# IRFM/librir

Hardware: AMD Instinct MI355X
Metric: IR frames/sec encode+decode, 640x512 uint16 (higher is better)
Workload: dtype u16; 1 GPU; configs[1]: 1000-frame 640x512 uint16 stream (S1 noisy background, seed 1234+rank), lossless RIRB1 encode+decode, device-resident, GOP 50, per GPU; two launches per step: the encoder leaves the PACKED form (headers + position and length per segment + the payload without holes: encoded_footprint_bytes, in a buffer of half the raw size), the decoder reads it as it is; the compressed payload (17 % of; frames_per_gpu=1000, width=640, height=512, gop=50

## Files before the change

### librir_amd/csrc/codec_kernels.hip

```cpp
#include <hip/hip_runtime.h>
#include <algorithm>
#include <stdint.h>

#include "codec_format.h"
#include "filter_kernels.h"
#include "runtime.h"

namespace rir
{

	constexpr int FRAME_LOAD_AUX = 2;
	constexpr int FRAME_STORE_AUX = 2;
	constexpr int SPARSE_STORE_AUX = 0;
	constexpr int STREAM_LOAD_AUX = 0;

	typedef short short2v __attribute__((ext_vector_type(2)));
	typedef unsigned short ushort2v __attribute__((ext_vector_type(2)));

	__device__ __forceinline__ uint32_t pk_sub16(uint32_t a, uint32_t b)
	{
		return __builtin_bit_cast(uint32_t, __builtin_bit_cast(ushort2v, a) - __builtin_bit_cast(ushort2v, b));
	}
	__device__ __forceinline__ uint32_t pk_add16(uint32_t a, uint32_t b)
	{
// ... 306 lines not shown
		v = max(v, (uint32_t)__builtin_amdgcn_mov_dpp((int)v, 0x121, 0xf, 0xf, false));
		v = max(v, (uint32_t)__builtin_amdgcn_mov_dpp((int)v, 0x122, 0xf, 0xf, false));
		v = max(v, (uint32_t)__builtin_amdgcn_mov_dpp((int)v, 0x124, 0xf, 0xf, false));
		v = max(v, (uint32_t)__builtin_amdgcn_mov_dpp((int)v, 0x128, 0xf, 0xf, false));
		return v;
	}
	__device__ __forceinline__ uint32_t rows_inclusive_sum(uint32_t w)
	{
		const uint32_t s = w + (uint32_t)__builtin_amdgcn_update_dpp(0, (int)w, 0x142, 0xa, 0xf, false);
		return s + (uint32_t)__builtin_amdgcn_update_dpp(0, (int)s, 0x143, 0xc, 0xf, false);
	}

	__device__ __forceinline__ uint32_t half_inclusive_sum(uint32_t v)
	{
		v += (uint32_t)__builtin_amdgcn_update_dpp(0, (int)v, 0x111, 0xf, 0xf, true);
		v += (uint32_t)__builtin_amdgcn_update_dpp(0, (int)v, 0x112, 0xf, 0xf, true);
		v += (uint32_t)__builtin_amdgcn_update_dpp(0, (int)v, 0x114, 0xf, 0xf, true);
		v += (uint32_t)__builtin_amdgcn_update_dpp(0, (int)v, 0x118, 0xf, 0xf, true);
		v += (uint32_t)__builtin_amdgcn_update_dpp(0, (int)v, 0x142, 0xa, 0xf, false);
		return v;
	}
	__device__ __forceinline__ uint32_t bitlen_nz(uint32_t f) { return 31u - (uint32_t)__builtin_clz((f << 1) | 1u); }

	struct RecordWords
	{
		v2u32 va, vb;
		uint32_t pa, pb;
	};

	template <uint32_t SCALE, uint32_t NONE>
	__device__ __forceinline__ uint64_t emit_words_narrow(const Px8 &r, uint32_t mode, uint32_t base, RecordWords &rw, uint32_t pos,
														  const LaneConsts &lc, const TransposeConsts &tc, uint32_t *words)
	{
		uint32_t x = (r.d[0] | (r.d[1] << 8)) | ((r.d[2] | (r.d[3] << 8)) << 4);
		x = transpose32(x, tc);
		const uint64_t nz64 = __ballot(x != 0);
		const uint32_t nz = (uint32_t)nz64 | (uint32_t)(nz64 >> 32);
		uint32_t M = nz | ((nz >> 1) & 0x77777777u);
		M |= (M >> 2) & 0x33333333u;
		uint32_t W = M - ((M >> 1) & 0x55555555u);
		W = (W & 0x33333333u) + ((W >> 2) & 0x33333333u);
		*words = (uint32_t)__builtin_popcount(M);
		auto sw = __builtin_amdgcn_permlane32_swap(x, x, false, false);
		rw.va.x = x, rw.va.y = sw[1];
		const uint32_t at = (pos + (uint32_t)__builtin_popcount(M & lc.p_before)) * SCALE;
		rw.pa = __builtin_amdgcn_inverse_ballot_w64((uint64_t)M) ? at : NONE;
		rw.vb = rw.va, rw.pb = NONE;
		const uint32_t B = base | (mode << 16);
		const uint64_t hw = __ballot((int32_t)(W << lc.p_hshw) < 0) & 0x00E700E700E700E7ull;
		const uint64_t hb = __ballot((int32_t)(B << lc.p_hshb) < 0) & 0x3C003C003C00FC00ull;
		return hw | hb;
	}

	template <uint32_t SCALE, uint32_t NONE>
	__device__ __forceinline__ uint64_t emit_words_wide(const Px8 &r, uint32_t mode, uint32_t base, RecordWords &rw, uint32_t pos,
														const LaneConsts &lc, const TransposeConsts &tc, uint32_t *words)
	{
		uint32_t alo = r.d[0], ahi = r.d[1], blo = r.d[2], bhi = r.d[3];
		transpose64x2(alo, ahi, blo, bhi, tc);
		const uint32_t wa = row_allmax((alo | ahi) != 0 ? lc.bitp1 : 0u);
		const uint32_t wb = row_allmax((blo | bhi) != 0 ? lc.bitp1 : 0u);
		const uint32_t ia = rows_inclusive_sum(wa), ib = rows_inclusive_sum(wb);
		const uint32_t tot_a = (uint32_t)__builtin_amdgcn_readlane((int)ia, 63);
		const uint32_t tot_b = (uint32_t)__builtin_amdgcn_readlane((int)ib, 63);
		rw.va.x = alo, rw.va.y = ahi, rw.vb.x = blo, rw.vb.y = bhi;
		rw.pa = lc.bit < wa ? (pos + ia - wa + lc.bit) * SCALE : NONE;
		rw.pb = lc.bit < wb ? (pos + tot_a + ib - wb + lc.bit) * SCALE : NONE;
		*words = tot_a + tot_b;
		const uint32_t nib = (base >> lc.sh4) & 15u;
		const uint32_t field = ((nib << 10) | (lc.row0 ? mode << 14 : 0u)) | ((wb << 5) | wa);
		return __ballot((field & lc.onehot) != 0);
	}

	template <uint32_t SCALE, uint32_t NONE>
	__device__ __forceinline__ uint64_t emit_words(const Px8 &r, uint32_t mode, uint32_t base, RecordWords &rw, uint32_t pos, const LaneConsts &lc,
												   const TransposeConsts &tc, uint32_t *words)
	{
		const uint32_t any = (r.d[0] | r.d[1]) | (r.d[2] | r.d[3]);
		if (__ballot((any & 0xfff0fff0u) != 0) == 0)
			return emit_words_narrow<SCALE, NONE>(r, mode, base, rw, pos, lc, tc, words);
		return emit_words_wide<SCALE, NONE>(r, mode, base, rw, pos, lc, tc, words);
	}

	struct DirectSink
	{
		__amdgpu_buffer_rsrc_t out;
		template <int DIR>
		__device__ __forceinline__ uint64_t emit(const Px8 &r, uint32_t mode, uint32_t base, uint32_t pos, const LaneConsts &lc,
												 const TransposeConsts &tc, uint32_t *words)
		{
			static_assert(DIR > 0, "a slot is filled in frame order from word 0: the direct sink only walks forwards");
			RecordWords rw;
			const uint64_t h = emit_words<8u, RIR_OOB>(r, mode, base, rw, pos, lc, tc, words);
			__builtin_amdgcn_raw_buffer_store_b64(rw.va, out, rw.pa, 0, SPARSE_STORE_AUX);
			__builtin_amdgcn_raw_buffer_store_b64(rw.vb, out, rw.pb, 0, SPARSE_STORE_AUX);
			return h;
		}
	};

	__device__ __noinline__ uint64_t staging_take_extent(unsigned long long *cursor, uint32_t need, uint64_t arena_words, uint32_t *error_word)
	{
		unsigned long long off = 0;
		if ((threadIdx.x & 63u) == 0)
			off = __hip_atomic_fetch_add(cursor, (unsigned long long)need, __ATOMIC_RELAXED, __HIP_MEMORY_SCOPE_AGENT);
		const uint32_t lo = (uint32_t)__builtin_amdgcn_readfirstlane((int)(uint32_t)off);
		const uint32_t hi = (uint32_t)__builtin_amdgcn_readfirstlane((int)(uint32_t)(off >> 32));
		off = ((unsigned long long)hi << 32) | lo;
		if (off + need > arena_words)
		{
			if ((threadIdx.x & 63u) == 0)
				__hip_atomic_fetch_or(error_word, 2u, __ATOMIC_RELAXED, __HIP_MEMORY_SCOPE_AGENT);
			return ~0ull;
		}
		return off;
	}

	struct Staging
	{
		uint64_t *lds;
		uint32_t cap;
		uint32_t lds_used;
		bool spilling;
		__amdgpu_buffer_rsrc_t spill;
		uint32_t need;
		uint64_t *arena;
		unsigned long long *cursor;
		uint64_t arena_words;
		uint64_t extent;
		uint32_t *error_word;

		__device__ __forceinline__ Staging(uint64_t *lds_all, int w, int cap_, int nrec)
			: lds(lds_all + (size_t)w * cap_), cap((uint32_t)cap_), lds_used(0), spilling(false), need((uint32_t)(nrec > 0 ? nrec : 0) * RIRB1_REC_MAX_WORDS),
			  arena(nullptr), cursor(nullptr), arena_words(0), extent(~0ull), error_word(nullptr)
		{
		}

		template <int DIR>
		__device__ __forceinline__ uint64_t emit(const Px8 &r, uint32_t mode, uint32_t base, uint32_t pos, const LaneConsts &lc, const TransposeConsts &tc,
												 uint32_t *words)
		{
			RecordWords rw;
			const uint64_t h = emit_words<1u, RIR_NONE>(r, mode, base, rw, DIR > 0 ? pos : 0u, lc, tc, words);
			if (!spilling && pos + *words > cap)
			{
				spilling = true, lds_used = pos;
				if (arena)
				{
					const uint64_t ext = staging_take_extent(cursor, need, arena_words, error_word);
					extent = ((uint64_t)(uint32_t)__builtin_amdgcn_readfirstlane((int)(uint32_t)(ext >> 32)) << 32) |
							 (uint32_t)__builtin_amdgcn_readfirstlane((int)(uint32_t)ext);
					if (extent != ~0ull)
						spill = make_rsrc(arena + extent, need * 8u);
				}
			}
			if (!spilling)
			{
				uint64_t *rec = DIR > 0 ? lds : lds + (cap - pos - *words);
				if (rw.pa != RIR_NONE)
					rec[rw.pa] = ((uint64_t)rw.va.y << 32) | rw.va.x;
				if (rw.pb != RIR_NONE)
					rec[rw.pb] = ((uint64_t)rw.vb.y << 32) | rw.vb.x;
			}
			const uint32_t add = !spilling ? RIR_OOB : DIR > 0 ? 0u - lds_used * 8u : (need - (pos - lds_used) - *words) * 8u;
			const uint32_t oa = rw.pa != RIR_NONE ? rw.pa * 8u + add : RIR_OOB;
			const uint32_t ob = rw.pb != RIR_NONE ? rw.pb * 8u + add : RIR_OOB;
			__builtin_amdgcn_raw_buffer_store_b64(rw.va, spill, oa, 0, SPARSE_STORE_AUX);
			__builtin_amdgcn_raw_buffer_store_b64(rw.vb, spill, ob, 0, SPARSE_STORE_AUX);
			return h;
		}
	};

	template <bool FAST, int DIR, class Sink>
	__device__ __forceinline__ uint32_t encode_run(const uint16_t *__restrict__ frames, int64_t npx, int nload, int64_t frame_first, bool has_key,
												   int tile, int lane, uint64_t *__restrict__ hdr_first, Sink &sink)
	{
		constexpr bool BACK = DIR < 0;
		const int64_t p0 = (int64_t)tile * RIRB1_TILE_PX + lane * 8;
		const TransposeConsts tc = make_transpose_consts(lane);
		const LaneConsts lc = make_lane_consts(lane);
		const uint32_t lane_off = (uint32_t)lane * 16u;
		const uint16_t *next_ptr = frames + (frame_first + (BACK ? nload - 1 : 0)) * npx + (int64_t)tile * RIRB1_TILE_PX;
		auto load = [&](int k, v4u32 &dst) {
			if (FAST)
			{
				const Px8 p = buf_load8(next_ptr, k < nload ? lane_off : RIR_OOB);
				dst.x = p.d[0], dst.y = p.d[1], dst.z = p.d[2], dst.w = p.d[3];
				next_ptr = BACK ? next_ptr - npx : next_ptr + npx;
			}
			else
			{
				const int i = min(k, nload - 1);
				const Px8 p = load8(frames, frame_first + (BACK ? nload - 1 - i : i), npx, p0, false);
				dst.x = p.d[0], dst.y = p.d[1], dst.z = p.d[2], dst.w = p.d[3];
			}
		};
		auto as_px8 = [](const v4u32 &v) {
			Px8 p;
			p.d[0] = v.x, p.d[1] = v.y, p.d[2] = v.z, p.d[3] = v.w;
			return p;
		};
		uint32_t pos = 0;
		uint64_t hdr_reg = 0;
		auto key_record = [&](const Px8 &cur) {
			const uint32_t base_raw = tile_base(cur, false);
			const uint32_t b2 = base_raw | (base_raw << 16);
			Px8 r_raw;
#pragma unroll
			for (int k = 0; k < 4; ++k)
				r_raw.d[k] = pk_sub16(cur.d[k], b2);
			const Px8 dl = left_delta(cur, lane);
			const uint32_t base_left = tile_base(dl, true);
			const uint32_t bl2 = base_left | (base_left << 16);
			Px8 r_left;
#pragma unroll
			for (int k = 0; k < 4; ++k)
				r_left.d[k] = pk_sub16(dl.d[k], bl2);
			const bool use_left = payload_words(r_left) < payload_words(r_raw);
			Px8 r_sel;
#pragma unroll
			for (int k = 0; k < 4; ++k)
				r_sel.d[k] = use_left ? r_left.d[k] : r_raw.d[k];
			uint32_t words;
			const uint32_t key_mode = use_left ? RIRB1_MODE_LEFT : RIRB1_MODE_RAW;
			const uint64_t h = sink.template emit<DIR>(r_sel, key_mode, use_left ? base_left : base_raw, pos, lc, tc, &words);
			if (lane == 0)
				hdr_first[0] = h;
			pos += words;
		};
		v4u32 s0, s1, s2, s3;
		load(0, s0);
		load(1, s1);
		load(2, s2);
		load(3, s3);
		if (!BACK && has_key)
			key_record(as_px8(s0));
#define RIR_ENC_STEP(K, NEW, OLD)                                                             \
	{                                                                                          \
		const int k_ = (K);                                                                    \
		Px8 d;                                                                                 \
		{                                                                                      \
			const Px8 c_ = as_px8(BACK ? OLD : NEW), p_ = as_px8(BACK ? NEW : OLD);            \
			_Pragma("unroll") for (int k = 0; k < 4; ++k) d.d[k] = pk_sub16(c_.d[k], p_.d[k]); \
		}                                                                                      \
		load(k_ + 3, OLD);                                                                     \
		const uint32_t base = tile_base(d, true);                                              \
		const uint32_t b2 = base | (base << 16);                                               \
		_Pragma("unroll") for (int k = 0; k < 4; ++k) d.d[k] = pk_sub16(d.d[k], b2);          \
		uint32_t words;                                                                        \
		const uint64_t h = sink.template emit<DIR>(d, RIRB1_MODE_TEMPORAL, base, pos, lc, tc, &words); \
		if (lane == ((k_ - 1) & 63))                                                           \
			hdr_reg = h;                                                                       \
		pos += words;                                                                          \
	}
		int fb = 1;
		while (fb < nload)
		{
			const int g0 = fb, gend = min(fb + 64, nload);
			for (; fb + 3 < gend; fb += 4)
			{
				RIR_ENC_STEP(fb, s1, s0)
				RIR_ENC_STEP(fb + 1, s2, s1)
				RIR_ENC_STEP(fb + 2, s3, s2)
				RIR_ENC_STEP(fb + 3, s0, s3)
			}
			if (fb < gend)
			{
				RIR_ENC_STEP(fb, s1, s0)
				if (fb + 1 < gend)
				{
					RIR_ENC_STEP(fb + 1, s2, s1)
					if (fb + 2 < gend)
						RIR_ENC_STEP(fb + 2, s3, s2)
				}
				fb = gend;
			}
			if (g0 + lane < gend)
				hdr_first[BACK ? nload - (g0 + lane) : g0 + lane] = hdr_reg;
			hdr_reg = 0;
		}
#undef RIR_ENC_STEP
		if (BACK && has_key)
		{
			const int ks = (nload - 1) & 3;
			const v4u32 kv = ks == 0 ? s0 : ks == 1 ? s1 : ks == 2 ? s2 : s3;
			key_record(as_px8(kv));
		}
		return pos;
	}

	template <bool FAST>
	__attribute__((amdgpu_waves_per_eu(8, 8))) __global__ __launch_bounds__(256) void rirb1_encode_tiles(const uint16_t *__restrict__ frames, int64_t npx, int ntiles,
																 int tile_first, int tile_count, int nframes, int gop,
																 uint64_t *__restrict__ hdr_table, uint32_t *__restrict__ seg_words,
																 uint64_t *__restrict__ sparse)
	{
		const int lane = threadIdx.x & 63;
		const int ti = blockIdx.x * 4 + __builtin_amdgcn_readfirstlane((int)(threadIdx.x >> 6));
		if (ti >= tile_count)
			return;
		const int tile = tile_first + ti;
		const int chunk = blockIdx.y;
		const int f_begin = chunk * gop;
		const int nf = min(gop, nframes - f_begin);
		const int64_t slot = (int64_t)chunk * ntiles + tile;
		uint64_t *my_hdr = hdr_table + slot * gop;
		DirectSink sink{make_rsrc(sparse + slot * RIRB1_SLOT_WORDS(gop), (uint32_t)gop * RIRB1_REC_MAX_WORDS * 8u)};
		const uint32_t words = encode_run<FAST, 1>(frames, npx, nf, f_begin, true, tile, lane, my_hdr, sink);
		for (int f = nf + lane; f < gop; f += 64)
			my_hdr[f] = 0;
		if (lane == 0)
			seg_words[slot] = words;
	}

	__global__ __launch_bounds__(256) void rirb1_scan_tiles(const uint32_t *__restrict__ seg_words, int ntiles,
														   uint32_t *__restrict__ tile_off, uint64_t *__restrict__ chunk_words)
	{
		__shared__ uint32_t wave_tot[4];
		__shared__ uint32_t carry_s;
		const int c = blockIdx.x, tid = threadIdx.x, lane = tid & 63, wv = tid >> 6;
		const uint32_t *in = seg_words + (int64_t)c * ntiles;
		uint32_t *off = tile_off + (int64_t)c * (ntiles + 1);
		if (tid == 0)
			carry_s = 0;
		__syncthreads();
		for (int base = 0; base < ntiles; base += 256)
		{
			const int i = base + tid;
			const uint32_t v = i < ntiles ? in[i] : 0u;
			const uint32_t inc = wave_scan_add(v, lane);
			if (lane == 63)
				wave_tot[wv] = inc;
			__syncthreads();
			uint32_t pre = carry_s;
			for (int k = 0; k < wv; ++k)
				pre += wave_tot[k];
			if (i < ntiles)
				off[i] = pre + inc - v;
			__syncthreads();
			if (tid == 255)
				carry_s = pre + inc;
			__syncthreads();
		}
		if (tid == 0)
		{
			off[ntiles] = carry_s;
			chunk_words[c] = carry_s;
		}
	}

	__global__ __launch_bounds__(256) void rirb1_compact(const uint64_t *__restrict__ sparse, const uint32_t *__restrict__ tile_off,
														const uint64_t *__restrict__ chunk_words, int ntiles, int nchunks, int gop,
														uint64_t *__restrict__ chunk_off, uint64_t *__restrict__ stream)
	{
		const int t = blockIdx.x, c = blockIdx.y, tid = threadIdx.x;
		const uint32_t *off = tile_off + (int64_t)c * (ntiles + 1);
		const uint32_t o0 = off[t], o1 = off[t + 1];
		uint64_t s = 0;
		for (int i = tid & 63; i < c; i += 64)
			s += chunk_words[i];
#pragma unroll
		for (int d = 32; d >= 1; d >>= 1)
			s += (uint64_t)__shfl_xor((long long)s, d, 64);
// ... 311 lines not shown
		const int f_begin = chunk * gop;
		const int nf = min(gop, nframes - f_begin);
		uint64_t *my_hdr = hdr_table + seg * gop;

		const WaveShare sh = wave_share<enc_split_mirrored>(w, WAVES, nf);
		Staging sg(enc_lds, w, cap, sh.nrec);
		sg.spill = make_rsrc(arena, 0);
		sg.arena = arena, sg.cursor = spill_cursor, sg.arena_words = arena_words, sg.error_word = error_word;
		uint32_t pos = 0;
		if (sh.nrec > 0)
		{
			if (enc_walks_back(w))
				pos = encode_run<FAST, -1>(frames, npx, sh.nload, (int64_t)f_begin + sh.first_load, sh.has_key, tile, lane, my_hdr + sh.first_load, sg);
			else
				pos = encode_run<FAST, 1>(frames, npx, sh.nload, (int64_t)f_begin + sh.first_load, sh.has_key, tile, lane, my_hdr + sh.first_load, sg);
		}
		if (lane == 0)
			sh_u64[1 + w] = sg.extent;
		staged_publish<WAVES>(my_hdr, nf, gop, sg, pos, w, lane, sh_u32, sh_u32 + WAVES);
		__syncthreads();
		if (w != 0)
			return;
		uint32_t total = 0;
		bool lost = false;
#pragma unroll
		for (int i = 0; i < WAVES; ++i)
		{
			const uint32_t n = sh_u32[i];
			total += n;
			lost |= n > sh_u32[WAVES + i] && sh_u64[1 + i] == ~0ull;
		}
		unsigned long long at = 0;
		if (lane == 0)
			at = __hip_atomic_fetch_add(cursor, (unsigned long long)total | (1ull << RIR_PACKED_COUNT_SHIFT), __ATOMIC_RELAXED, __HIP_MEMORY_SCOPE_AGENT);
		const uint32_t lo = (uint32_t)__builtin_amdgcn_readfirstlane((int)(uint32_t)at);
		const uint32_t hi = (uint32_t)__builtin_amdgcn_readfirstlane((int)(uint32_t)(at >> 32));
		const uint32_t arrived = hi >> (RIR_PACKED_COUNT_SHIFT - 32);
		const uint64_t nseg = (uint64_t)gridDim.y * (uint32_t)ntiles;
		const uint64_t on_side = downwards ? nseg / 2 : (nseg + 1) / 2;
		if ((uint64_t)arrived + 1 == on_side)
			packed_finish(ctrl, capacity_words, nseg < 2 ? 1u : 2u);
		at = ((unsigned long long)hi << 32 | lo) & RIR_PACKED_WORDS_MASK;
		const bool fits = at + total <= capacity_words;
		if (downwards)
			at = capacity_words - at - total;
		if (lane == 0)
		{
			seg_pos[seg] = at;
			seg_words[seg] = total;
			sh_u64[0] = (fits && !lost) ? at : ~0ull;
		}
		if (!fits || lost)
			return;
		uint64_t *dst = stream + at;
		for (int i = 0; i < WAVES; ++i)
		{
			const uint32_t n_all = sh_u32[i];
			copy_wave_words(dst, enc_lds + (size_t)i * cap, (uint32_t)cap, n_all, sh_u32[WAVES + i], enc_walks_back(i), lane, [&](uint32_t &need) {
				need = (uint32_t)wave_share<enc_split_mirrored>(i, WAVES, nf).nrec * RIRB1_REC_MAX_WORDS;
				return make_rsrc(arena + sh_u64[1 + i], need * 8u);
			});
			dst += n_all;
		}
	}

	struct Fetched
	{
		uint64_t hdr;
		v2u32 a, b;
		uint32_t words;
		bool bad;
		bool narrow;
	};

	__device__ __forceinline__ bool header_is_narrow(uint64_t hdr)
	{
		const uint64_t m0 = 0x0021002100210021ull;
		const uint64_t hi = hdr & (m0 * 0x18u);
		const uint64_t b2 = (hdr >> 2) & m0;
		const uint64_t lo = (hdr | (hdr >> 1)) & m0;
		return (hi | (b2 & lo)) == 0;
	}

	__device__ __forceinline__ Fetched fetch_record(uint64_t hdr, __amdgpu_buffer_rsrc_t in, uint32_t pos, uint32_t seg_len, const LaneConsts &lc)
	{
		Fetched r;
		r.hdr = hdr;
		r.narrow = header_is_narrow(hdr);
		const bool hdr_bad = ((hdr & 0xC000C000C0000000ull) != 0) || (((hdr >> 14) & 3u) == 3u);
		uint32_t oa, ob;
		if (r.narrow)
		{
			const uint32_t w = ((lc.n_hhi ? (uint32_t)(hdr >> 32) : (uint32_t)hdr) >> lc.n_hsh) & 31u;
			const uint32_t incl = half_inclusive_sum(lc.n_first ? w : 0u);
			r.words = (uint32_t)__builtin_amdgcn_readlane((int)incl, 31);
			r.bad = hdr_bad || (pos + r.words > seg_len);
			oa = (!r.bad && lc.n_half == 0 && lc.n_bit < w) ? (pos + incl - w + lc.n_bit) * 8u : RIR_OOB;
			ob = RIR_OOB;
		}
		else
		{
			const uint32_t field = ((lc.row_hi ? (uint32_t)(hdr >> 32) : (uint32_t)hdr) >> lc.sh16) & 0xffffu;
			const uint32_t wa = field & 31u, wb = (field >> 5) & 31u;
			const uint32_t ia = rows_inclusive_sum(wa), ib = rows_inclusive_sum(wb);
			const uint32_t tot_a = (uint32_t)__builtin_amdgcn_readlane((int)ia, 63);
			const uint32_t tot_b = (uint32_t)__builtin_amdgcn_readlane((int)ib, 63);
			r.words = tot_a + tot_b;
			const bool too_wide = __ballot(wa > 16u || wb > 16u) != 0;
			r.bad = hdr_bad || too_wide || (pos + r.words > seg_len);
			oa = (!r.bad && lc.bit < wa) ? (pos + ia - wa + lc.bit) * 8u : RIR_OOB;
			ob = (!r.bad && lc.bit < wb) ? (pos + tot_a + ib - wb + lc.bit) * 8u : RIR_OOB;
		}
		r.a = __builtin_amdgcn_raw_buffer_load_b64(in, oa, 0, STREAM_LOAD_AUX);
		r.b = __builtin_amdgcn_raw_buffer_load_b64(in, ob, 0, STREAM_LOAD_AUX);
		return r;
	}

	__device__ __forceinline__ Px8 planes_to_residuals(v2u32 a, v2u32 b, bool narrow, const TransposeConsts &tc)
	{
		Px8 r;
		if (narrow)
		{
			auto sw = __builtin_amdgcn_permlane32_swap(a.x, a.y, false, false);
			const uint32_t x = transpose32(sw[0], tc);
			const uint32_t lo = x & 0x0f0f0f0fu, hi = (x >> 4) & 0x0f0f0f0fu;
			r.d[0] = __builtin_amdgcn_perm(hi, lo, 0x0c040c00u);
			r.d[1] = __builtin_amdgcn_perm(hi, lo, 0x0c050c01u);
			r.d[2] = __builtin_amdgcn_perm(hi, lo, 0x0c060c02u);
			r.d[3] = __builtin_amdgcn_perm(hi, lo, 0x0c070c03u);
		}
		else
		{
			uint32_t alo = a.x, ahi = a.y, blo = b.x, bhi = b.y;
			transpose64x2(alo, ahi, blo, bhi, tc);
			r.d[0] = alo, r.d[1] = ahi, r.d[2] = blo, r.d[3] = bhi;
		}
		return r;
	}

	__device__ __forceinline__ uint64_t readlane64(uint64_t v, int l)
	{
		return (uint64_t)(uint32_t)__builtin_amdgcn_readlane((int)(uint32_t)v, l) |
			   ((uint64_t)(uint32_t)__builtin_amdgcn_readlane((int)(uint32_t)(v >> 32), l) << 32);
	}

	__device__ __forceinline__ Px8 left_integrate(const Px8 &d, int lane)
	{
		uint32_t a[8];
#pragma unroll
		for (int k = 0; k < 4; ++k)
		{
			a[2 * k] = d.d[k] & 0xffffu;
			a[2 * k + 1] = d.d[k] >> 16;
		}
#pragma unroll
		for (int i = 1; i < 8; ++i)
			a[i] = (a[i] + a[i - 1]) & 0xffffu;
		const uint32_t incl = wave_scan_add(a[7], lane);
		const uint32_t carry = (incl - a[7]) & 0xffffu;
		Px8 o;
#pragma unroll
		for (int k = 0; k < 4; ++k)
			o.d[k] = ((a[2 * k] + carry) & 0xffffu) | (((a[2 * k + 1] + carry) & 0xffffu) << 16);
		return o;
	}

	struct ChunkSink
	{
		uint16_t *frames, *tile0;
		int64_t npx, frame0, p0;
		uint32_t lane_off;
		__device__ __forceinline__ ChunkSink(uint16_t *frames_, int64_t npx_, int64_t frame0_, int tile, int lane)
			: frames(frames_), tile0(frames_ + frame0_ * npx_ + (int64_t)tile * RIRB1_TILE_PX), npx(npx_), frame0(frame0_),
			  p0((int64_t)tile * RIRB1_TILE_PX + lane * 8), lane_off((uint32_t)lane * 16u)
		{
		}
		template <bool FAST>
		__device__ __forceinline__ void put(int f, const Px8 &o)
		{
			if (FAST)
				buf_store8(tile0 + (int64_t)f * npx, lane_off, o);
			else
				store8(frames, frame0 + f, npx, p0, false, o);
		}
	};

	template <bool FAST, class Sink>
	__device__ __forceinline__ void decode_tile(const uint64_t *__restrict__ my_hdr, const uint64_t *__restrict__ in_ptr, uint32_t seg_len,
												int nf, bool check_end, int lane, Sink &sink, int *__restrict__ error_flag)
	{
		const TransposeConsts tc = make_transpose_consts(lane);
		const LaneConsts lc = make_lane_consts(lane);
		const __amdgpu_buffer_rsrc_t in = make_rsrc(in_ptr, seg_len * 8u);

		Px8 prev;
		prev.d[0] = prev.d[1] = prev.d[2] = prev.d[3] = 0;
		uint32_t pos = 0;
		bool err = false;
		for (int f0 = 0; f0 < nf; f0 += 64)
		{
			const int nr = min(64, nf - f0);
			const uint64_t my_h = lane < nr ? my_hdr[f0 + lane] : 0ull;
			Fetched r0 = fetch_record(readlane64(my_h, 0), in, pos, seg_len, lc);
			pos += r0.words;
			Fetched r1 = fetch_record(nr > 1 ? readlane64(my_h, 1) : 0ull, in, pos, seg_len, lc);
			pos += r1.words;
			Fetched r2 = fetch_record(nr > 2 ? readlane64(my_h, 2) : 0ull, in, pos, seg_len, lc);
			pos += r2.words;
			Fetched r3 = fetch_record(nr > 3 ? readlane64(my_h, 3) : 0ull, in, pos, seg_len, lc);
			pos += r3.words;
#define RIR_DEC_STEP(FR, R)                                                                                          \
	if ((FR) < nr)                                                                                                   \
	{                                                                                                                \
		const int fr = (FR);                                                                                         \
		const uint64_t hdr = R.hdr;                                                                                  \
		err |= R.bad;                                                                                                \
		const v2u32 wa_ = R.a, wb_ = R.b;                                                                             \
		const bool narrow_ = R.narrow;                                                                               \
		                                                       \
		R = fetch_record(fr + 4 < nr ? readlane64(my_h, fr + 4) : 0ull, in, pos, seg_len, lc);                        \
		pos += R.words;                                                                                              \
		const Px8 res = planes_to_residuals(wa_, wb_, narrow_, tc);                                                  \
		const uint32_t mode = (uint32_t)(hdr >> 14) & 3u;                                                            \
		const uint32_t base = ((uint32_t)(hdr >> 10) & 0xfu) | ((uint32_t)(hdr >> 22) & 0xf0u) |                     \
							  ((uint32_t)(hdr >> 34) & 0xf00u) | ((uint32_t)(hdr >> 46) & 0xf000u);                  \
		const uint32_t b2 = base | (base << 16);                                                                     \
		Px8 o;                                                                                                       \
		_Pragma("unroll") for (int k = 0; k < 4; ++k) o.d[k] = pk_add16(res.d[k], b2);                              \
		if (f0 + fr == 0)                                                                                            \
		{                                                                                \
			if (mode == RIRB1_MODE_LEFT)                                                                             \
				o = left_integrate(o, lane);                                                                         \
			err |= (mode == RIRB1_MODE_TEMPORAL);                                                                    \
		}                                                                                                            \
		else                                                                                                         \
		{                                                \
			const uint32_t keep = (mode == RIRB1_MODE_TEMPORAL) ? 0xffffffffu : 0u;                                  \
			_Pragma("unroll") for (int k = 0; k < 4; ++k) o.d[k] = pk_add16(prev.d[k] & keep, o.d[k]);              \
			err |= (mode == RIRB1_MODE_LEFT);                                                                        \
		}                                                                                                            \
		sink.template put<FAST>(f0 + fr, o);                                                                         \
		prev = o;                                                                                                    \
	}
			for (int fb = 0; fb < nr; fb += 4)
			{
				RIR_DEC_STEP(fb, r0)
				RIR_DEC_STEP(fb + 1, r1)
				RIR_DEC_STEP(fb + 2, r2)
				RIR_DEC_STEP(fb + 3, r3)
			}
#undef RIR_DEC_STEP
		}
		if ((err || (check_end && pos != seg_len)) && lane == 0)
			atomicExch(error_flag, 1);
	}

	__global__ __launch_bounds__(256) void rirb1_decode_tiles(const uint64_t *__restrict__ hdr_table, const uint32_t *__restrict__ tile_off,
															 const uint64_t *__restrict__ chunk_off, const uint64_t *__restrict__ stream,
															 uint64_t stream_words, int64_t npx, int ntiles, int nframes, int gop,
															 const int64_t *__restrict__ chunk_frames, const uint32_t *__restrict__ seg_words,
															 uint16_t *__restrict__ frames, int *__restrict__ error_flag)
	{
		const int lane = threadIdx.x & 63;
		const int tile = blockIdx.x * 4 + __builtin_amdgcn_readfirstlane((int)(threadIdx.x >> 6));
		if (tile >= ntiles)
			return;
		const int chunk = blockIdx.y;
		int64_t f_begin = (int64_t)chunk * gop;
		int nf = (int)min((int64_t)gop, (int64_t)nframes - f_begin);
		if (chunk_frames)
		{
			const int64_t cf = chunk_frames[2 * chunk], cn = chunk_frames[2 * chunk + 1];
			if (cn == 0)
				return;
			if (cf < 0 || cn < 0 || cn > gop || cf > (int64_t)nframes - cn)
			{
				if (lane == 0)
					atomicExch(error_flag, 1);
				return;
			}
			f_begin = cf, nf = (int)cn;
		}
		const int64_t slot = (int64_t)chunk * ntiles + tile;
		const uint64_t *my_hdr = hdr_table + slot * gop;
		uint32_t seg_len;
		const uint64_t *in;
		if (seg_words)
		{
			const uint64_t base = (uint64_t)slot * (uint64_t)RIRB1_SLOT_WORDS(gop);
			seg_len = min(seg_words[slot], (uint32_t)gop * RIRB1_REC_MAX_WORDS);
			if (base > stream_words || (uint64_t)seg_len > stream_words - base)
			{
				if (lane == 0)
					atomicExch(error_flag, 1);
				return;
			}
			in = stream + base;
		}
		else
		{
			const uint32_t t0 = tile_off[(int64_t)chunk * (ntiles + 1) + tile];
			const uint32_t t1 = tile_off[(int64_t)chunk * (ntiles + 1) + tile + 1];
			const uint64_t c0 = chunk_off[chunk], c1 = chunk_off[chunk + 1];
			if (c0 > c1 || c1 > stream_words || t1 < t0 || (uint64_t)t1 > c1 - c0)
			{
				if (lane == 0)
					atomicExch(error_flag, 1);
				return;
			}
			seg_len = min(t1 - t0, (uint32_t)gop * RIRB1_REC_MAX_WORDS);
			in = stream + c0 + t0;
		}
		const bool fast = ((npx & 7) == 0) && ((int64_t)(tile + 1) * RIRB1_TILE_PX <= npx) && ((((uintptr_t)frames) & 15) == 0);
		ChunkSink sink(frames, npx, f_begin, tile, lane);
		if (fast)
			decode_tile<true>(my_hdr, in, seg_len, nf, true, lane, sink, error_flag);
		else
			decode_tile<false>(my_hdr, in, seg_len, nf, true, lane, sink, error_flag);
	}

	template <bool FAST>
	__attribute__((amdgpu_waves_per_eu(8, 8))) __global__ __launch_bounds__(256) void rirb1_decode_packed(
		const uint64_t *__restrict__ hdr_table, const uint64_t *__restrict__ seg_pos, const uint32_t *__restrict__ seg_words,
		const uint64_t *__restrict__ stream, uint64_t stream_words, int64_t npx, int ntiles, int tile0, int tile_end, int nframes, int gop,
		uint16_t *__restrict__ frames, int *__restrict__ error_flag)
	{
		const int lane = threadIdx.x & 63;
		const int tile = tile0 + blockIdx.x * 4 + __builtin_amdgcn_readfirstlane((int)(threadIdx.x >> 6));
		if (tile >= tile_end)
			return;
		const int chunk = blockIdx.y;
		const int64_t f_begin = (int64_t)chunk * gop;
		const int nf = (int)min((int64_t)gop, (int64_t)nframes - f_begin);
		const int64_t slot = (int64_t)chunk * ntiles + tile;
		const uint64_t base = seg_pos[slot];
		const uint32_t seg_len = min(seg_words[slot], (uint32_t)gop * RIRB1_REC_MAX_WORDS);
		if (base > stream_words || (uint64_t)seg_len > stream_words - base)
		{
			if (lane == 0)
				atomicExch(error_flag, 1);
			return;
		}
		ChunkSink sink(frames, npx, f_begin, tile, lane);
		decode_tile<FAST>(hdr_table + slot * gop, stream + base, seg_len, nf, true, lane, sink, error_flag);
	}

	template <bool F32>
	struct SelectSink
	{
		char *cur;
		int64_t fbytes;
		int next, step;
		int npx, p0;
		uint32_t lane_off, min_t;
		int nmin;
		__device__ __forceinline__ Px8 add_min(Px8 o) const
		{
			if (min_t)
			{
#pragma unroll
				for (int k = 0; k < 4; ++k)
					o.d[k] = pk_add16(o.d[k], (2 * k < nmin ? min_t : 0u) | (2 * k + 1 < nmin ? min_t << 16 : 0u));
			}
			return o;
		}
		template <bool FAST>
		__device__ __forceinline__ void put(int f, const Px8 &r)
		{
			const bool sel = f == next;
			const Px8 o = add_min(r);
			if (FAST)
			{
				if (F32)
				{
					v4u32 a, b;
					a.x = __builtin_bit_cast(uint32_t, (float)(o.d[0] & 0xffffu)), a.y = __builtin_bit_cast(uint32_t, (float)(o.d[0] >> 16));
					a.z = __builtin_bit_cast(uint32_t, (float)(o.d[1] & 0xffffu)), a.w = __builtin_bit_cast(uint32_t, (float)(o.d[1] >> 16));
					b.x = __builtin_bit_cast(uint32_t, (float)(o.d[2] & 0xffffu)), b.y = __builtin_bit_cast(uint32_t, (float)(o.d[2] >> 16));
					b.z = __builtin_bit_cast(uint32_t, (float)(o.d[3] & 0xffffu)), b.w = __builtin_bit_cast(uint32_t, (float)(o.d[3] >> 16));
					const __amdgpu_buffer_rsrc_t r4 = make_rsrc(cur, RIRB1_TILE_PX * 4);
					__builtin_amdgcn_raw_buffer_store_b128(a, r4, sel ? lane_off * 2u : RIR_OOB, 0, FRAME_STORE_AUX);
					__builtin_amdgcn_raw_buffer_store_b128(b, r4, sel ? lane_off * 2u + 16u : RIR_OOB, 0, FRAME_STORE_AUX);
				}
				else
				{
					v4u32 v;
					v.x = o.d[0], v.y = o.d[1], v.z = o.d[2], v.w = o.d[3];
					__builtin_amdgcn_raw_buffer_store_b128(v, make_rsrc(cur, RIRB1_TILE_PX * 2), sel ? lane_off : RIR_OOB, 0, FRAME_STORE_AUX);
				}
			}
			else if (sel)
			{
#pragma unroll
				for (int k = 0; k < 8; ++k)
				{
					const uint32_t v = (o.d[k >> 1] >> (16 * (k & 1))) & 0xffffu;
					if (p0 + k < npx)
					{
						if (F32)
							reinterpret_cast<float *>(cur)[lane_off / 2u + k] = (float)v;
						else
							reinterpret_cast<uint16_t *>(cur)[lane_off / 2u + k] = (uint16_t)v;
					}
				}
			}
			if (sel)
				next += step, cur += fbytes;
		}
	};

	template <bool F32, bool FAST>
	__attribute__((amdgpu_waves_per_eu(8, 8))) __global__ __launch_bounds__(256) void rirb1_decode_select(
		const uint64_t *__restrict__ hdr_table, const uint32_t *__restrict__ tile_off, const uint64_t *__restrict__ chunk_off, const uint64_t *__restrict__ stream,
		uint64_t stream_words, int64_t npx, int ntiles, int tile0, int tile_end, int gop, int nchunks, const RirbSelect *__restrict__ table, int out_frames,
		void *__restrict__ out, int min_px, uint32_t min_t, int *__restrict__ error_flag)
	{
		const int lane = threadIdx.x & 63;
		const int tile = tile0 + blockIdx.x * 4 + __builtin_amdgcn_readfirstlane((int)(threadIdx.x >> 6));
		if (tile >= tile_end)
			return;
		const RirbSelect e = table[blockIdx.y];
		if (e.count == 0)
			return;
		const int64_t walk = (int64_t)e.first + (int64_t)(e.count - 1) * e.step + 1;
		if (e.chunk < 0 || e.chunk >= nchunks || e.nframes <= 0 || e.nframes > gop || e.first < 0 || e.count < 0 || e.step < 1 || walk > e.nframes ||
			e.out_first < 0 || e.out_first > out_frames - e.count)
		{
			if (lane == 0)
				atomicExch(error_flag, 1);
			return;
		}
		const int chunk = e.chunk;
		const uint32_t t0 = tile_off[(int64_t)chunk * (ntiles + 1) + tile];
		const uint32_t t1 = tile_off[(int64_t)chunk * (ntiles + 1) + tile + 1];
		const uint64_t c0 = chunk_off[chunk], c1 = chunk_off[chunk + 1];
		if (c0 > c1 || c1 > stream_words || t1 < t0 || (uint64_t)t1 > c1 - c0)
		{
			if (lane == 0)
				atomicExch(error_flag, 1);
			return;
		}
		const uint32_t seg_len = min(t1 - t0, (uint32_t)gop * RIRB1_REC_MAX_WORDS);
		const int tpx = tile * RIRB1_TILE_PX;
		SelectSink<F32> sink;
		sink.fbytes = npx * (F32 ? 4 : 2);
		sink.cur = static_cast<char *>(out) + (int64_t)e.out_first * sink.fbytes + (int64_t)tpx * (F32 ? 4 : 2);
		sink.next = e.first, sink.step = e.step;
		sink.npx = (int)npx, sink.p0 = tpx + lane * 8;
		sink.lane_off = (uint32_t)lane * 16u, sink.min_t = min_t & 0xffffu;
		sink.nmin = max(0, min(8, min_px - sink.p0));
		decode_tile<FAST>(hdr_table + ((int64_t)chunk * ntiles + tile) * gop, stream + c0 + t0, seg_len, (int)walk, walk == e.nframes, lane, sink, error_flag);
	}


	template <class KFast, class KRagged, class Launch>
	static void launch_fast_then_ragged(const void *frames, int64_t npx, int ntiles, KFast fast, KRagged ragged, Launch launch)
	{
		const bool aligned = ((npx & 7) == 0) && ((((uintptr_t)frames) & 15) == 0);
		const int nfast = aligned ? (int)std::min<int64_t>(ntiles, npx / RIRB1_TILE_PX) : 0;
		if (nfast > 0)
			launch(fast, 0, nfast);
		if (ntiles > nfast)
			launch(ragged, nfast, ntiles);
	}

	static int staged_lds_words(int gop, int waves)
	{
		const int share = (gop + 1 + waves - 1) / waves + 1;
		return std::min(448 * 4 / waves, share * RIRB1_REC_MAX_WORDS);
	}

	hipError_t launch_encode_tiles(const uint16_t *d_frames, int64_t npx, int ntiles, int nframes, int gop, uint64_t *d_hdr,
								   uint32_t *d_seg_words, uint64_t *d_sparse, hipStream_t st)
	{
		const int nchunks = (nframes + gop - 1) / gop;
		launch_fast_then_ragged(d_frames, npx, ntiles, rirb1_encode_tiles<true>, rirb1_encode_tiles<false>, [&](auto kernel, int t0, int t1) {
			hipLaunchKernelGGL(kernel, dim3((t1 - t0 + 3) / 4, nchunks), dim3(256), 0, st, d_frames, npx, ntiles, t0, t1 - t0, nframes, gop, d_hdr, d_seg_words,
							   d_sparse);
		});
		return hipGetLastError();
	}

	hipError_t launch_encode_compact(int ntiles, int nframes, int gop, const uint32_t *d_seg_words, const uint64_t *d_sparse,
									 uint32_t *d_tile_off, uint64_t *d_chunk_words, uint64_t *d_chunk_off, uint64_t *d_stream, hipStream_t st)
	{
		const int nchunks = (nframes + gop - 1) / gop;
		dim3 block(256);
		hipLaunchKernelGGL(rirb1_scan_tiles, dim3(nchunks), block, 0, st, d_seg_words, ntiles, d_tile_off, d_chunk_words);
		hipLaunchKernelGGL(rirb1_compact, dim3(ntiles, nchunks), block, 0, st, d_sparse, d_tile_off, d_chunk_words, ntiles, nchunks, gop,
						   d_chunk_off, d_stream);
		return hipGetLastError();
// ... 95 lines not shown
```

Before: 3.826 million frames/s.

## Pad memory counters with dummy OOB stores and flatten encode/decode frame loops

Adds out-of-bounds dummy buffer stores in the encoder and decoder prologues, apparently so the store counter sits at a steady depth and the waitcnt pattern is uniform from the first iteration. The encoder's nested 64-frame group loop becomes one flat loop that flushes headers every 64 frames. The decoder drops per-group header readlanes, reads headers directly from memory one step ahead, and splits record fetch into a plan and an issue step so address computation happens before residual unpacking. This costs extra no-op stores and scalar or global header loads per frame, and changes the register schedule.

After: 3.833 million frames/s, median of 6. Within noise of the previous version (+0.2%).

```diff
diff --git a/librir_amd/csrc/codec_kernels.hip b/librir_amd/csrc/codec_kernels.hip
--- a/librir_amd/csrc/codec_kernels.hip
+++ b/librir_amd/csrc/codec_kernels.hip
@@ -412,6 +412,14 @@
 		return emit_words_wide<SCALE, NONE>(r, mode, base, rw, pos, lc, tc, words);
 	}
 
+	__device__ __forceinline__ void pad_stores(__amdgpu_buffer_rsrc_t rsrc)
+	{
+		v2u32 z;
+		z.x = 0, z.y = 0;
+		__builtin_amdgcn_raw_buffer_store_b64(z, rsrc, RIR_OOB, 0, SPARSE_STORE_AUX);
+		__builtin_amdgcn_raw_buffer_store_b64(z, rsrc, RIR_OOB + 256u, 0, SPARSE_STORE_AUX);
+	}
+
 	struct DirectSink
 	{
 		__amdgpu_buffer_rsrc_t out;
@@ -426,6 +434,7 @@
 			__builtin_amdgcn_raw_buffer_store_b64(rw.vb, out, rw.pb, 0, SPARSE_STORE_AUX);
 			return h;
 		}
+		__device__ __forceinline__ void pad() const { pad_stores(out); }
 	};
 
 	__device__ __noinline__ uint64_t staging_take_extent(unsigned long long *cursor, uint32_t need, uint64_t arena_words, uint32_t *error_word)
@@ -498,6 +507,7 @@
 			__builtin_amdgcn_raw_buffer_store_b64(rw.vb, spill, ob, 0, SPARSE_STORE_AUX);
 			return h;
 		}
+		__device__ __forceinline__ void pad() const { pad_stores(spill); }
 	};
 
 	template <bool FAST, int DIR, class Sink>
@@ -560,8 +570,14 @@
 		v4u32 s0, s1, s2, s3;
 		load(0, s0);
 		load(1, s1);
+		if (FAST)
+			sink.pad();
 		load(2, s2);
+		if (FAST)
+			sink.pad();
 		load(3, s3);
+		if (FAST)
+			sink.pad();
 		if (!BACK && has_key)
 			key_record(as_px8(s0));
 #define RIR_ENC_STEP(K, NEW, OLD)                                                             \
@@ -582,32 +598,32 @@
 			hdr_reg = h;                                                                       \
 		pos += words;                                                                          \
 	}
-		int fb = 1;
-		while (fb < nload)
-		{
-			const int g0 = fb, gend = min(fb + 64, nload);
-			for (; fb + 3 < gend; fb += 4)
-			{
-				RIR_ENC_STEP(fb, s1, s0)
+		int fb = 1, g0 = 1;
+		for (; fb + 3 < nload; fb += 4)
+		{
+			RIR_ENC_STEP(fb, s1, s0)
+			RIR_ENC_STEP(fb + 1, s2, s1)
+			RIR_ENC_STEP(fb + 2, s3, s2)
+			RIR_ENC_STEP(fb + 3, s0, s3)
+			if (fb + 4 - g0 == 64)
+			{
+				hdr_first[BACK ? nload - (g0 + lane) : g0 + lane] = hdr_reg;
+				hdr_reg = 0;
+				g0 += 64;
+			}
+		}
+		if (fb < nload)
+		{
+			RIR_ENC_STEP(fb, s1, s0)
+			if (fb + 1 < nload)
+			{
 				RIR_ENC_STEP(fb + 1, s2, s1)
-				RIR_ENC_STEP(fb + 2, s3, s2)
-				RIR_ENC_STEP(fb + 3, s0, s3)
-			}
-			if (fb < gend)
-			{
-				RIR_ENC_STEP(fb, s1, s0)
-				if (fb + 1 < gend)
-				{
-					RIR_ENC_STEP(fb + 1, s2, s1)
-					if (fb + 2 < gend)
-						RIR_ENC_STEP(fb + 2, s3, s2)
-				}
-				fb = gend;
-			}
-			if (g0 + lane < gend)
-				hdr_first[BACK ? nload - (g0 + lane) : g0 + lane] = hdr_reg;
-			hdr_reg = 0;
-		}
+				if (fb + 2 < nload)
+					RIR_ENC_STEP(fb + 2, s3, s2)
+			}
+		}
+		if (g0 + lane < nload)
+			hdr_first[BACK ? nload - (g0 + lane) : g0 + lane] = hdr_reg;
 #undef RIR_ENC_STEP
 		if (BACK && has_key)
 		{
@@ -1085,9 +1101,15 @@
 		return (hi | (b2 & lo)) == 0;
 	}
 
-	__device__ __forceinline__ Fetched fetch_record(uint64_t hdr, __amdgpu_buffer_rsrc_t in, uint32_t pos, uint32_t seg_len, const LaneConsts &lc)
+	struct Planned
 	{
 		Fetched r;
+		uint32_t oa, ob;
+	};
+	__device__ __forceinline__ Planned plan_record(uint64_t hdr, uint32_t pos, uint32_t seg_len, const LaneConsts &lc)
+	{
+		Planned p;
+		Fetched &r = p.r;
 		r.hdr = hdr;
 		r.narrow = header_is_narrow(hdr);
 		const bool hdr_bad = ((hdr & 0xC000C000C0000000ull) != 0) || (((hdr >> 14) & 3u) == 3u);
@@ -1114,9 +1136,19 @@
 			oa = (!r.bad && lc.bit < wa) ? (pos + ia - wa + lc.bit) * 8u : RIR_OOB;
 			ob = (!r.bad && lc.bit < wb) ? (pos + tot_a + ib - wb + lc.bit) * 8u : RIR_OOB;
 		}
-		r.a = __builtin_amdgcn_raw_buffer_load_b64(in, oa, 0, STREAM_LOAD_AUX);
-		r.b = __builtin_amdgcn_raw_buffer_load_b64(in, ob, 0, STREAM_LOAD_AUX);
+		p.oa = oa, p.ob = ob;
+		return p;
+	}
+	__device__ __forceinline__ Fetched issue_record(const Planned &p, __amdgpu_buffer_rsrc_t in)
+	{
+		Fetched r = p.r;
+		r.a = __builtin_amdgcn_raw_buffer_load_b64(in, p.oa, 0, STREAM_LOAD_AUX);
+		r.b = __builtin_amdgcn_raw_buffer_load_b64(in, p.ob, 0, STREAM_LOAD_AUX);
 		return r;
+	}
+	__device__ __forceinline__ Fetched fetch_record(uint64_t hdr, __amdgpu_buffer_rsrc_t in, uint32_t pos, uint32_t seg_len, const LaneConsts &lc)
+	{
+		return issue_record(plan_record(hdr, pos, seg_len, lc), in);
 	}
 
 	__device__ __forceinline__ Px8 planes_to_residuals(v2u32 a, v2u32 b, bool narrow, const TransposeConsts &tc)
@@ -1186,6 +1218,12 @@
 			else
 				store8(frames, frame0 + f, npx, p0, false, o);
 		}
+		template <bool FAST>
+		__device__ __forceinline__ void pad()
+		{
+			if (FAST)
+				buf_store8(tile0, RIR_OOB, Px8{});
+		}
 	};
 
 	template <bool FAST, class Sink>
@@ -1200,37 +1238,45 @@
 		prev.d[0] = prev.d[1] = prev.d[2] = prev.d[3] = 0;
 		uint32_t pos = 0;
 		bool err = false;
-		for (int f0 = 0; f0 < nf; f0 += 64)
-		{
-			const int nr = min(64, nf - f0);
-			const uint64_t my_h = lane < nr ? my_hdr[f0 + lane] : 0ull;
-			Fetched r0 = fetch_record(readlane64(my_h, 0), in, pos, seg_len, lc);
+		if (nf > 0)
+		{
+			auto header = [&](int q) {
+				const uint64_t h = my_hdr[min(q, nf - 1)];
+				return q < nf ? h : 0ull;
+			};
+			Fetched r0 = fetch_record(header(0), in, pos, seg_len, lc);
 			pos += r0.words;
-			Fetched r1 = fetch_record(nr > 1 ? readlane64(my_h, 1) : 0ull, in, pos, seg_len, lc);
+			Fetched r1 = fetch_record(header(1), in, pos, seg_len, lc);
 			pos += r1.words;
-			Fetched r2 = fetch_record(nr > 2 ? readlane64(my_h, 2) : 0ull, in, pos, seg_len, lc);
+			sink.template pad<FAST>();
+			Fetched r2 = fetch_record(header(2), in, pos, seg_len, lc);
 			pos += r2.words;
-			Fetched r3 = fetch_record(nr > 3 ? readlane64(my_h, 3) : 0ull, in, pos, seg_len, lc);
+			sink.template pad<FAST>();
+			Fetched r3 = fetch_record(header(3), in, pos, seg_len, lc);
 			pos += r3.words;
-#define RIR_DEC_STEP(FR, R)                                                                                          \
-	if ((FR) < nr)                                                                                                   \
+			sink.template pad<FAST>();
+			uint64_t h_ahead = header(4);
+#define RIR_DEC_STEP(FR, R, KEY, AHEAD)                                                                              \
 	{                                                                                                                \
 		const int fr = (FR);                                                                                         \
 		const uint64_t hdr = R.hdr;                                                                                  \
 		err |= R.bad;                                                                                                \
-		const v2u32 wa_ = R.a, wb_ = R.b;                                                                             \
-		const bool narrow_ = R.narrow;                                                                               \
-		                                                       \
-		R = fetch_record(fr + 4 < nr ? readlane64(my_h, fr + 4) : 0ull, in, pos, seg_len, lc);                        \
-		pos += R.words;                                                                                              \
-		const Px8 res = planes_to_residuals(wa_, wb_, narrow_, tc);                                                  \
+		 \
+		 \
+		 \
+		const Planned ahead_ = plan_record(h_ahead, pos, seg_len, lc);                                               \
+		pos += ahead_.r.words;                                                                                       \
+		h_ahead = (AHEAD);                                                                                           \
+		const Px8 res = planes_to_residuals(R.a, R.b, R.narrow, tc);                                                 \
+		         \
+		R = issue_record(ahead_, in);                                                                                \
 		const uint32_t mode = (uint32_t)(hdr >> 14) & 3u;                                                            \
 		const uint32_t base = ((uint32_t)(hdr >> 10) & 0xfu) | ((uint32_t)(hdr >> 22) & 0xf0u) |                     \
 							  ((uint32_t)(hdr >> 34) & 0xf00u) | ((uint32_t)(hdr >> 46) & 0xf000u);                  \
 		const uint32_t b2 = base | (base << 16);                                                                     \
 		Px8 o;                                                                                                       \
 		_Pragma("unroll") for (int k = 0; k < 4; ++k) o.d[k] = pk_add16(res.d[k], b2);                              \
-		if (f0 + fr == 0)                                                                                            \
+		if (KEY)                                                                                                     \
 		{                                                                                \
 			if (mode == RIRB1_MODE_LEFT)                                                                             \
 				o = left_integrate(o, lane);                                                                         \
@@ -1242,15 +1288,27 @@
 			_Pragma("unroll") for (int k = 0; k < 4; ++k) o.d[k] = pk_add16(prev.d[k] & keep, o.d[k]);              \
 			err |= (mode == RIRB1_MODE_LEFT);                                                                        \
 		}                                                                                                            \
-		sink.template put<FAST>(f0 + fr, o);                                                                         \
+		sink.template put<FAST>(fr, o);                                                                              \
 		prev = o;                                                                                                    \
 	}
-			for (int fb = 0; fb < nr; fb += 4)
-			{
-				RIR_DEC_STEP(fb, r0)
-				RIR_DEC_STEP(fb + 1, r1)
-				RIR_DEC_STEP(fb + 2, r2)
-				RIR_DEC_STEP(fb + 3, r3)
+			RIR_DEC_STEP(0, r0, true, header(5))
+			int fb = 1;
+			for (; fb + 3 < nf; fb += 4)
+			{
+				RIR_DEC_STEP(fb, r1, false, header(fb + 5))
+				RIR_DEC_STEP(fb + 1, r2, false, header(fb + 6))
+				RIR_DEC_STEP(fb + 2, r3, false, header(fb + 7))
+				RIR_DEC_STEP(fb + 3, r0, false, header(fb + 8))
+			}
+			if (fb < nf)
+			{
+				RIR_DEC_STEP(fb, r1, false, 0ull)
+				if (fb + 1 < nf)
+				{
+					RIR_DEC_STEP(fb + 1, r2, false, 0ull)
+					if (fb + 2 < nf)
+						RIR_DEC_STEP(fb + 2, r3, false, 0ull)
+				}
 			}
 #undef RIR_DEC_STEP
 		}
@@ -1410,6 +1468,19 @@
 			if (sel)
 				next += step, cur += fbytes;
 		}
+		template <bool FAST>
+		__device__ __forceinline__ void pad()
+		{
+			if (FAST)
+			{
+				const __amdgpu_buffer_rsrc_t r4 = make_rsrc(cur, RIRB1_TILE_PX * 2);
+				v4u32 z;
+				z.x = z.y = z.z = z.w = 0;
+				__builtin_amdgcn_raw_buffer_store_b128(z, r4, RIR_OOB, 0, FRAME_STORE_AUX);
+				if (F32)
+					__builtin_amdgcn_raw_buffer_store_b128(z, r4, RIR_OOB + 256u, 0, FRAME_STORE_AUX);
+			}
+		}
 	};
 
 	template <bool F32, bool FAST>
```
